# tkoolen/Parametron.jl

Hardware: AMD Instinct MI355X
Metric: QP re-evaluations/sec (Q,q,C,d rebuild) at n=4096 (higher is better)
Workload: dtype f64; 1 GPU; C2 dense least-squares QP: n=4096 vars, A 4096x4096, m=512 equality rows, fp64; canonical Q,q,const + C,d MOI triplets; n=4096, r=4096, m=512, objective_mode=canonical, instances_per_gpu=1, parallelism=single GPU, replay=tape

## Files before the change

### parametron.jl_amd/csrc/gram_mid.hip

```cpp
#include "affine_tile.h"
#include "gram_common.h"

#ifndef PMT_MID_WPS
#define PMT_MID_WPS 1
#endif
#ifndef PMT_MID_G
#define PMT_MID_G 256
#endif
#ifndef PMT_MID_MAXWG
#define PMT_MID_MAXWG 2304
#endif
#ifndef PMT_MID_D
#define PMT_MID_D 2
#endif
#ifndef PMT_MID_GROUP_US
#define PMT_MID_GROUP_US 1.15
#endif
#ifndef PMT_MID_TAIL_US
#define PMT_MID_TAIL_US 0.95
#endif
#ifndef PMT_MID_SB
#define PMT_MID_SB 8
#endif
#ifndef PMT_MID_FB
#define PMT_MID_FB 4
#endif
#ifndef PMT_MID_FORMAL
#if defined(__HIP_DEVICE_COMPILE__) && !defined(__gfx950__) && !defined(__gfx942__)
#define PMT_MID_FORMAL 1
#else
#define PMT_MID_FORMAL 0
#endif
#endif

#ifdef PMT_MID_TRACE
__device__ unsigned long long g_mid_trace[1024 * 8];
__device__ unsigned long long g_mid_walk[1024 * 8];
__device__ unsigned long long g_mid_riders[1024 * 2];
#define MID_TRACE_WORDS 8
__device__ __forceinline__ void mid_walk_note(unsigned long long *w, int k, unsigned long long t) {
    if (k == 0) { if (w[0]) w[4] += t - w[7]; else w[5] = t; w[0] += 1; }
    else if (k == 1) w[1] += t - w[7];
    else if (k == 3 || k == 5) { w[2] += t - w[7]; w[6] = t; }
    else if (k == 6) { w[3] += t - w[7]; w[6] = t; }
    else return;
    w[7] = t;
}
#define MID_STAMP(k) do { if (threadIdx.x == 0 && blockIdx.x < 1024) { const unsigned long long t_ = wall_clock64(); g_mid_trace[blockIdx.x * 8 + (k)] = t_; \
                          mid_walk_note(reinterpret_cast<unsigned long long *>(sh + MSH), (k), t_); } } while (0)
extern "C" int pmt_mid_trace_read(unsigned long long *host) {
    return hipMemcpyFromSymbol(host, HIP_SYMBOL(g_mid_trace), sizeof(unsigned long long) * 1024 * 8) == hipSuccess ? 0 : 1;
}
extern "C" int pmt_mid_walk_read(unsigned long long *host) {
    return hipMemcpyFromSymbol(host, HIP_SYMBOL(g_mid_walk), sizeof(unsigned long long) * 1024 * 8) == hipSuccess ? 0 : 1;
}
extern "C" int pmt_mid_riders_read(unsigned long long *host) {
    return hipMemcpyFromSymbol(host, HIP_SYMBOL(g_mid_riders), sizeof(unsigned long long) * 1024 * 2) == hipSuccess ? 0 : 1;
}
#else
#define MID_STAMP(k) do { } while (0)
#define MID_TRACE_WORDS 0
#endif

namespace pmt {

constexpr int MT = 64;
constexpr int MACC = 64;
constexpr int MPART = MACC * 64;
constexpr int MSTRIDE = MPART + MT + 8;
constexpr int MPITCH = MT + 1;
constexpr int MFG = 8;
constexpr int MCNT = 16;
constexpr int MQBUF = 4 * 2048;
constexpr int MFLAG = MQBUF + 4 * MT;
constexpr int MMAPS = MFLAG + 8;
constexpr int MSH = MMAPS + 2 * MT;

struct MidArgs {
    const double *A; int64_t lda, rows, cols;
    const double *b; int sign;
    const int64_t *xvar; const int64_t *varmap; int moi;
    QT *out_quad; double *out_csc; double alpha; LT *out_lin; double *out_const;
    int nb;
    int n_off, s_off, s_diag;
    int gpc_off, gpc_diag;
    int n_tail, s_tail, gpc_tail;
    double *ws;
    unsigned *counters;
    int xcd;
    int persist, total;
    unsigned *tickets;
    const AffineRider *riders;
    int nriders, rider_tiles;
};

struct MidPlan { int nb, n_off, s_off, s_diag, gpc_off, gpc_diag, n_tail, s_tail, gpc_tail, wgs; };

static double mid_fold_us(int count) { return 0.5 + 2.6 * (double)cdiv(count, PMT_MID_FB); }

static MidPlan mid_plan(int64_t rows, int64_t cols) {
    MidPlan p;
    p.nb = (int)cdiv(cols, MT);
    p.n_off = p.nb * (p.nb - 1) / 2;
    const int ngroups = (int)std::max<int64_t>(1, cdiv(rows, 8));
    const int maxs = std::max(1, ngroups / 4);
    auto sd = [&](int s) { return std::min(maxs, std::max(1, (5 * s + 7) / 8)); };
    int best = 1;
    double best_t = 1e300;
    for (int s = 1; s <= std::min(maxs, 64); ++s) {
        const int64_t wgs = (int64_t)p.n_off * s + (int64_t)p.nb * sd(s);
        if (s > 1 && wgs > PMT_MID_MAXWG) break;
        const double it_off = (double)cdiv(cdiv(ngroups, s), 4), it_diag = 0.69 * (double)cdiv(cdiv(ngroups, sd(s)), 4);
        const double fold = s <= 1 ? 0.0 : s <= MFG ? mid_fold_us(s) : mid_fold_us(MFG) + 1.5 + mid_fold_us((int)cdiv(s, MFG));
        const double t = (double)cdiv(wgs, PMT_MID_G) * (PMT_MID_GROUP_US * (p.n_off ? std::max(it_off, it_diag) : it_diag) + 5.0 + (s > 1 ? 1.0 : 0.0)) +
                         fold * (1.0 + (double)(p.n_off + p.nb) / PMT_MID_G);
        if (t < best_t) { best_t = t; best = s; }
    }
    int s = best;
#ifdef PMT_TUNING
    if (const char *e = getenv("PMT_MID_S")) { const int v = atoi(e); if (v > 0) s = std::min(v, maxs); }
#endif
    int sdiag = sd(s), ntail = 0, stail = 1;
    if (p.n_off + p.nb > PMT_MID_G) {
        auto wg_us = [&](int c, double w) { return PMT_MID_TAIL_US * w * (double)cdiv(cdiv(ngroups, c), 4) + 5.0 + (c > 1 ? 1.0 : 0.0); };
        const int rem = p.n_off % PMT_MID_G;
        int ct = 1;
        double tail_off = 0.0;
        if (rem) {
            tail_off = 1e300;
            for (int c = 1; c <= std::min(maxs, MFG); ++c) {
                const double t = (double)cdiv((int64_t)rem * c, PMT_MID_G) * wg_us(c, 1.0) + (c > 1 ? mid_fold_us(c) : 0.0);
                if (t < tail_off) { tail_off = t; ct = c; }
            }
        }
        const int last = rem ? (int)(((int64_t)rem * ct) % PMT_MID_G) : 0, free_cus = last ? PMT_MID_G - last : 0;
        const double t_last = rem ? wg_us(ct, 1.0) : wg_us(1, 1.0);
        int cd = 1;
        double tail_diag = 1e300;
        for (int c = 1; c <= std::min(maxs, MFG); ++c) {
            const double t_d = wg_us(c, 0.69);
            const int64_t inside = (int64_t)free_cus * (int64_t)(t_last / t_d);
            const int64_t left = std::max<int64_t>(0, (int64_t)p.nb * c - inside);
            const double t = (double)cdiv(left, PMT_MID_G) * t_d + (c > 1 ? mid_fold_us(c) : 0.0);
            if (t < tail_diag) { tail_diag = t; cd = c; }
        }
        const double t1 = (double)(p.n_off / PMT_MID_G) * wg_us(1, 1.0) + tail_off + tail_diag;
        if (s == 1 || t1 * (PMT_MID_GROUP_US / PMT_MID_TAIL_US) < best_t) { s = 1; sdiag = cd; ntail = ct > 1 ? rem : 0; stail = ct > 1 ? ct : 1; }
    }
#ifdef PMT_TUNING
    if (const char *e = getenv("PMT_MID_TAIL")) { if (atoi(e) == 0) { ntail = 0; stail = 1; } }
#endif
    p.gpc_off = (int)cdiv(ngroups, s);
    p.s_off = (int)cdiv(ngroups, p.gpc_off);
    p.gpc_diag = (int)cdiv(ngroups, sdiag);
    p.s_diag = (int)cdiv(ngroups, p.gpc_diag);
    p.n_tail = ntail;
    p.gpc_tail = (int)cdiv(ngroups, stail);
    p.s_tail = ntail ? (int)cdiv(ngroups, p.gpc_tail) : 1;
    if (p.s_tail <= 1) { p.n_tail = 0; p.s_tail = 1; p.gpc_tail = ngroups; }
    p.wgs = (p.n_off - p.n_tail) * p.s_off + p.n_tail * p.s_tail + p.nb * p.s_diag + 1;
    return p;
}

template <bool DIAG, bool FAST>
__device__ __forceinline__ void mid_load(const MidArgs &g, int64_t row0, int lane, int64_t cj0, int64_t ck0, const unsigned (&voff)[DIAG ? 4 : 8],
                                         f64x2 (&buf)[DIAG ? 4 : 8], f64x2 &cb) {
    constexpr int NG = DIAG ? 4 : 8;
    const int lm = lane & 15, lk = lane >> 4;
    if (FAST) {
        const char *base = reinterpret_cast<const char *>(g.A + row0);
#pragma unroll
        for (int t = 0; t < NG; ++t) buf[t] = *reinterpret_cast<const f64x2 *>(base + voff[t]);
        cb.x = 0.0; cb.y = 0.0;
        if (DIAG && g.b) cb = *reinterpret_cast<const f64x2 *>(g.b + row0 + 2 * lk);
        return;
    }
    const int64_t row = row0 + 2 * lk;
    const bool r0 = row < g.rows, r1 = row + 1 < g.rows;
#pragma unroll
    for (int t = 0; t < NG; ++t) {
        const int64_t col = (t < 4 ? cj0 : ck0) + 16 * (t & 3) + lm;
        const bool cv = col < g.cols;
        const bool v0 = cv && r0, v1 = cv && r1;
        const double *p0 = g.A + (v0 ? col * g.lda + row : 0), *p1 = g.A + (v1 ? col * g.lda + row + 1 : 0);
        const double x = *p0, y = *p1;
        buf[t].x = v0 ? x : 0.0;
        buf[t].y = v1 ? y : 0.0;
    }
    cb.x = 0.0; cb.y = 0.0;
    if (DIAG && g.b) {
        const double x = g.b[r0 ? row : 0], y = g.b[r1 ? row + 1 : 0];
        cb.x = r0 ? x : 0.0;
        cb.y = r1 ? y : 0.0;
    }
}

template <bool DIAG>
__device__ __forceinline__ void mid_compute(double *__restrict__ rot, const f64x2 (&buf)[DIAG ? 4 : 8], const f64x2 &cb, int sign, int lane,
                                            double (&acc)[MACC], double (&qacc)[4]) {
    constexpr int BO = DIAG ? 0 : 4;
    const int lm = lane & 15, lrow = lane & 48;
#pragma unroll
    for (int t = 0; t < 4; ++t) *reinterpret_cast<f64x2 *>(rot + (t * 64 + lane) * 2) = buf[BO + t];
    f64x2 bv[4][4];
#pragma unroll
    for (int c = 0; c < 4; ++c) {
        bv[c][0] = buf[BO + c];
#pragma unroll
        for (int r = 1; r < 4; ++r) {
            bv[c][r] = *reinterpret_cast<const f64x2 *>(rot + (c * 64 + lrow + ((lm + 4 * r) & 15)) * 2);
        }
    }
    __builtin_amdgcn_sched_barrier(0);
    constexpr int NC = 4;
#pragma unroll
    for (int c = 0; c < NC; ++c)
#pragma unroll
        for (int tm = 0; tm < (DIAG ? c + 1 : 4); ++tm) {
            const int a = (tm * 4 + c) * 4;
            acc[a] = __builtin_amdgcn_mfma_f64_4x4x4f64(buf[tm].x, bv[c][0].x, acc[a], 0, 0, 0);
        }
#pragma unroll
    for (int c = 0; c < NC; ++c)
#pragma unroll
        for (int tm = 0; tm < (DIAG ? c + 1 : 4); ++tm) {
            const int a = (tm * 4 + c) * 4;
            acc[a] = __builtin_amdgcn_mfma_f64_4x4x4f64(buf[tm].y, bv[c][0].y, acc[a], 0, 0, 0);
        }
    __builtin_amdgcn_sched_barrier(0);
#pragma unroll
    for (int c = 0; c < NC; ++c) {
#pragma unroll
        for (int r = 1; r < 4; ++r)
#pragma unroll
            for (int tm = 0; tm < (DIAG ? c + 1 : 4); ++tm) {
                const int a = (tm * 4 + c) * 4 + r;
                acc[a] = __builtin_amdgcn_mfma_f64_4x4x4f64(buf[tm].x, bv[c][r].x, acc[a], 0, 0, 0);
            }
#pragma unroll
        for (int r = 1; r < 4; ++r)
#pragma unroll
            for (int tm = 0; tm < (DIAG ? c + 1 : 4); ++tm) {
                const int a = (tm * 4 + c) * 4 + r;
                acc[a] = __builtin_amdgcn_mfma_f64_4x4x4f64(buf[tm].y, bv[c][r].y, acc[a], 0, 0, 0);
            }
    }
    if (DIAG) {
        const double c0 = signed_const(cb.x, sign), c1 = signed_const(cb.y, sign);
#pragma unroll
        for (int t = 0; t < 4; ++t) qacc[t] = __builtin_amdgcn_mfma_f64_4x4x4f64(buf[t].x, c0, qacc[t], 0, 0, 0);
#pragma unroll
        for (int t = 0; t < 4; ++t) qacc[t] = __builtin_amdgcn_mfma_f64_4x4x4f64(buf[t].y, c1, qacc[t], 0, 0, 0);
    }
}

#define MID_SB() __builtin_amdgcn_sched_barrier(0)
template <bool DIAG>
__device__ __forceinline__ void mid_step(const MidArgs &g, double *__restrict__ rot, int64_t next_row0, const char *base_a, const char *base_b,
                                         unsigned (&voff)[DIAG ? 4 : 8], f64x2 (&buf)[DIAG ? 4 : 8], f64x2 &cb, int sign, int lane,
                                         double (&acc)[MACC], double (&qacc)[4]) {
    constexpr int BO = DIAG ? 0 : 4;
    const int lm = lane & 15, lrow = lane & 48, lk = lane >> 4;
    auto reload = [&](int t) {
        asm volatile("" : "+v"(voff[t]));
        buf[t] = *reinterpret_cast<const f64x2 *>((t < 4 ? base_a : base_b) + voff[t]);
    };
    f64x2 bv[4][4];
#pragma unroll
    for (int c = 0; c < 4; ++c) bv[c][0] = buf[BO + c];
    auto lds_op = [&](int i) {
        if (i < 4) *reinterpret_cast<f64x2 *>(rot + (i * 64 + lane) * 2) = buf[BO + i];
        else {
            const int c = (i - 4) / 3, r = 1 + (i - 4) % 3;
            bv[c][r] = *reinterpret_cast<const f64x2 *>(rot + (c * 64 + lrow + ((lm + 4 * r) & 15)) * 2);
        }
    };
    MID_SB();
    int k = 0;
#pragma unroll
    for (int pass = 0; pass < 2; ++pass)
#pragma unroll
        for (int c = 0; c < 4; ++c)
#pragma unroll
            for (int tm = 0; tm < (DIAG ? c + 1 : 4); ++tm) {
                const int a = (tm * 4 + c) * 4;
                acc[a] = __builtin_amdgcn_mfma_f64_4x4x4f64(pass ? buf[tm].y : buf[tm].x, pass ? bv[c][0].y : bv[c][0].x, acc[a], 0, 0, 0);
                if (k < 16) { MID_SB(); lds_op(k); MID_SB(); }
                ++k;
            }
    if (DIAG) {
        const double c0 = signed_const(cb.x, sign), c1 = signed_const(cb.y, sign);
#pragma unroll
        for (int t = 0; t < 4; ++t) qacc[t] = __builtin_amdgcn_mfma_f64_4x4x4f64(buf[t].x, c0, qacc[t], 0, 0, 0);
#pragma unroll
        for (int t = 0; t < 4; ++t) qacc[t] = __builtin_amdgcn_mfma_f64_4x4x4f64(buf[t].y, c1, qacc[t], 0, 0, 0);
        MID_SB();
        cb = *reinterpret_cast<const f64x2 *>((g.b ? g.b : g.A) + next_row0 + 2 * lk);
    }
    MID_SB();
    int nb = 0;
#pragma unroll
    for (int tm = 0; tm < 4; ++tm) {
#pragma unroll
        for (int pass = 0; pass < 2; ++pass)
#pragma unroll
            for (int c = (DIAG ? tm : 0); c < 4; ++c)
#pragma unroll
                for (int r = 1; r < 4; ++r) {
                    const int a = (tm * 4 + c) * 4 + r;
                    acc[a] = __builtin_amdgcn_mfma_f64_4x4x4f64(pass ? buf[tm].y : buf[tm].x, pass ? bv[c][r].y : bv[c][r].x, acc[a], 0, 0, 0);
                    if (!DIAG && nb < 4) { MID_SB(); reload(4 + nb); MID_SB(); ++nb; }
                }
        MID_SB();
        reload(tm);
        MID_SB();
    }
}

__host__ __device__ constexpr bool mid_used(bool diag, int a) { return !diag || (a >> 4) <= ((a >> 2) & 3); }

__device__ __forceinline__ void mid_pos(int lane, int a, int &row, int &col) {
    const int i = lane >> 4, b = (lane >> 2) & 3, j = lane & 3;
    row = 16 * (a >> 4) + 4 * b + i;
    col = 16 * ((a >> 2) & 3) + 4 * ((b + (a & 3)) & 3) + j;
}

__device__ __forceinline__ void mid_maps(const MidArgs &g, double *sh, int tid, int jb, int kb) {
    u64 *cmap = reinterpret_cast<u64 *>(sh + MMAPS);
    if (tid >= 2 * MT || (!g.out_quad && jb != kb)) return;
    const int64_t i = (tid < MT ? (int64_t)kb * MT + tid : (int64_t)jb * MT + tid - MT);
    const int64_t v = i < g.cols ? g.xvar[i] : 1;
    cmap[tid] = (u64)(g.moi ? map_var(g.varmap, v) : v);
}

__device__ __forceinline__ void mid_epilogue(const MidArgs &g, double *sh, int tid, int jb, int kb) {
    const int wave = tid >> 6, lane = tid & 63;
    const int64_t n = g.cols, j0 = (int64_t)jb * MT, k0 = (int64_t)kb * MT;
    double *tile = sh;
    const double *qfin = sh + MT * MPITCH;
    const u64 *cmap = reinterpret_cast<const u64 *>(sh + MMAPS);
    const u64 *rmap = cmap + MT;
    if (g.out_csc) {
        const int64_t j = j0 + lane;
#pragma unroll 4
        for (int col = wave; col < MT; col += 4) {
            const int64_t k = k0 + col;
            double c = tile[lane * MPITCH + col];
            if (g.moi || j != k) c = 2 * c;
            if (k < n && j <= k) g.out_csc[k * (k + 1) / 2 + j] = g.alpha * c;
        }
    }
    if (g.out_quad) {
        u64 *out = reinterpret_cast<u64 *>(g.out_quad);
        u64 *desc = reinterpret_cast<u64 *>(sh + MT * MPITCH + MT);
        if (tid < MT) {
            const int64_t j = j0 + tid;
            const int64_t kstart = j > k0 ? j : k0;
            const int64_t kend = (k0 + MT < n) ? k0 + MT : n;
            const int64_t nterms = (j < n && kend > kstart) ? kend - kstart : 0;
            desc[2 * tid] = (u64)(j * n - (j * (j - 1)) / 2 + (kstart - j)) * 3;
            desc[2 * tid + 1] = (u64)nterms | (u64)(kstart - k0) << 16 | (u64)(kstart == j ? 1 : 0) << 24;
        }
        __syncthreads();
        const bool moi = g.moi != 0;
        const int uwave = __builtin_amdgcn_readfirstlane(wave);
#pragma unroll 4
        for (int i = 0; i < MT / 4; ++i) {
            const int row = 4 * i + uwave;
            const u64 w0 = desc[2 * row], info = desc[2 * row + 1];
            const int nterms = (int)(info & 0xffff), coff = (int)((info >> 16) & 0xff);
            const bool dg = ((info >> 24) & 1) != 0;
            double c = tile[row * MPITCH + coff + lane];
            const u64 m = cmap[(coff + lane) & (MT - 1)], rv = rmap[row];
            if (moi || !(dg && lane == 0)) c = 2 * c;
            if (lane < nterms) {
                u64 *d = out + w0 + 3 * lane;
                d[0] = (u64)__double_as_longlong(c);
                d[1] = rv;
                d[2] = m;
            }
        }
    }
    if (jb == kb && tid < MT) {
        const int64_t j = j0 + tid;
        if (j < n) {
            LT t;
            t.coeff = 2 * qfin[tid];
            t.var = (int64_t)rmap[tid];
            g.out_lin[j] = t;
        }
    }
}

__device__ __forceinline__ void mid_constant(const MidArgs &g, double *sh, int tid) {
    const int wave = tid >> 6, lane = tid & 63;
    double s0 = 0.0, s1 = 0.0;
    if (g.b && g.sign) {
        for (int64_t i = tid; i < g.rows; i += 512) { const double c = signed_const(g.b[i], g.sign); s0 = s0 + c * c; }
        for (int64_t i = tid + 256; i < g.rows; i += 512) { const double c = signed_const(g.b[i], g.sign); s1 = s1 + c * c; }
    }
#pragma unroll
    for (int off = 32; off > 0; off >>= 1) { s0 = s0 + __shfl_down(s0, off, 64); s1 = s1 + __shfl_down(s1, off, 64); }
    if (lane == 0) { sh[wave] = s0; sh[4 + wave] = s1; }
    __syncthreads();
    if (tid == 0) {
        double v = sh[0];
#pragma unroll
        for (int w = 1; w < 8; ++w) v = v + sh[w];
        *g.out_const = v;
    }
}

__device__ __forceinline__ void mid_put(double *p, double v) {
#if PMT_MID_FORMAL
    *p = v;
#else
    __hip_atomic_store(p, v, __ATOMIC_RELAXED, __HIP_MEMORY_SCOPE_AGENT);
#endif
}
__device__ __forceinline__ double mid_get(const double *p) {
#if PMT_MID_FORMAL
    return *p;
#else
    return __hip_atomic_load(p, __ATOMIC_RELAXED, __HIP_MEMORY_SCOPE_AGENT);
#endif
}

template <bool DIAG, int W>
__device__ __forceinline__ void mid_tail(const MidArgs &g, double *sh, int lane, double (&acc)[MACC], const double (&qacc)[4], int nchunk, double *w) {
    constexpr int KEEP1 = (W >> 1) * 32, GIVE1 = 32 - KEEP1, KEEP2 = KEEP1 + (W & 1) * 16, GIVE2 = KEEP1 + 16 - (W & 1) * 16;
    double *mine = sh + W * 2048;
    const double *half = sh + (W ^ 2) * 2048, *quarter = sh + (W ^ 1) * 2048;
    const bool qlane = (lane & 3) == 0;
    const int qcol = 4 * ((lane >> 2) & 3) + (lane >> 4);
#pragma unroll
    for (int a = 0; a < 32; a += 2)
        if (mid_used(DIAG, GIVE1 + a)) { f64x2 v; v.x = acc[GIVE1 + a]; v.y = acc[GIVE1 + a + 1]; *reinterpret_cast<f64x2 *>(mine + (a * 32 + lane) * 2) = v; }
    if (DIAG && qlane) {
#pragma unroll
        for (int t = 0; t < 4; ++t) sh[MQBUF + W * MT + 16 * t + qcol] = qacc[t];
    }
    __syncthreads();
#pragma unroll
    for (int a = 0; a < 32; a += 2)
        if (mid_used(DIAG, KEEP1 + a)) {
            const f64x2 v = *reinterpret_cast<const f64x2 *>(half + (a * 32 + lane) * 2);
            acc[KEEP1 + a] = acc[KEEP1 + a] + v.x; acc[KEEP1 + a + 1] = acc[KEEP1 + a + 1] + v.y;
        }
    double qsum = 0.0;
    if (DIAG && W == 0) qsum = (sh[MQBUF + lane] + sh[MQBUF + 2 * MT + lane]) + (sh[MQBUF + MT + lane] + sh[MQBUF + 3 * MT + lane]);
    __syncthreads();
#pragma unroll
    for (int a = 0; a < 16; a += 2)
        if (mid_used(DIAG, GIVE2 + a)) { f64x2 v; v.x = acc[GIVE2 + a]; v.y = acc[GIVE2 + a + 1]; *reinterpret_cast<f64x2 *>(mine + (a * 32 + lane) * 2) = v; }
    __syncthreads();
#pragma unroll
    for (int a = 0; a < 16; a += 2)
        if (mid_used(DIAG, KEEP2 + a)) {
            const f64x2 v = *reinterpret_cast<const f64x2 *>(quarter + (a * 32 + lane) * 2);
            acc[KEEP2 + a] = acc[KEEP2 + a] + v.x; acc[KEEP2 + a + 1] = acc[KEEP2 + a + 1] + v.y;
        }
    __syncthreads();
    if (nchunk == 1) {
#pragma unroll
        for (int a = KEEP2; a < KEEP2 + 16; ++a) {
            if (!mid_used(DIAG, a)) continue;
            int row, col;
            mid_pos(lane, a, row, col);
            sh[row * MPITCH + col] = acc[a];
        }
        if (DIAG && W == 0) sh[MT * MPITCH + lane] = qsum;
        return;
    }
#pragma unroll
    for (int a = KEEP2; a < KEEP2 + 16; ++a) if (mid_used(DIAG, a)) mid_put(&w[a * 64 + lane], acc[a]);
    if (DIAG && W == 0) mid_put(&w[MPART + lane], qsum);
#if PMT_MID_FORMAL
    __builtin_amdgcn_fence(__ATOMIC_RELEASE, "agent");
#else
    __builtin_amdgcn_s_waitcnt(0);
#endif
}

template <bool DIAG>
__device__ __forceinline__ void mid_fold(const double *p, int count, int64_t stride, int tid, double (&sum)[16], double &qs) {
#pragma unroll
    for (int u = 0; u < 16; ++u) sum[u] = 0.0;
    qs = 0.0;
    for (int c0 = 0; c0 < count; c0 += PMT_MID_FB) {
        double v[PMT_MID_FB][16], qv[PMT_MID_FB];
#pragma unroll
        for (int cc = 0; cc < PMT_MID_FB; ++cc) {
            const double *pc = p + (int64_t)min(c0 + cc, count - 1) * stride;
#pragma unroll
            for (int u = 0; u < 16; ++u) {
                const int a = (tid >> 6) + 4 * u;
                v[cc][u] = 0.0;
                if (mid_used(DIAG, a)) v[cc][u] = mid_get(pc + tid + 256 * u);
            }
            qv[cc] = 0.0;
            if (DIAG && tid < MT) qv[cc] = mid_get(pc + MPART + tid);
        }
#pragma unroll
        for (int cc = 0; cc < PMT_MID_FB; ++cc) {
            const bool live = c0 + cc < count;
#pragma unroll
            for (int u = 0; u < 16; ++u) { const double t = sum[u] + v[cc][u]; sum[u] = live ? t : sum[u]; }
            const double t = qs + qv[cc];
            qs = live ? t : qs;
        }
    }
}

struct MidWalk {
    bool early;
    unsigned *ticket; int id0;
    int *slot;
    int drawn;
    bool next_full; int njb, nkb, nrank;
    bool pre;
};

template <int N>
__device__ __forceinline__ void mid_forget(f64x2 (&buf)[PMT_MID_D][N]) {
#pragma unroll
    for (int d = 0; d < PMT_MID_D; ++d)
#pragma unroll
        for (int t = 0; t < N; ++t) asm volatile("" : "=v"(buf[d][t].x), "=v"(buf[d][t].y));
}

template <bool DIAG>
__device__ __forceinline__ auto &mid_buf(f64x2 (&own)[PMT_MID_D][4], f64x2 (&walk)[PMT_MID_D][8]) {
    if constexpr (DIAG) return own; else return walk;
}

template <bool DIAG, bool FAST>
__device__ __forceinline__ void mid_body(const MidArgs &g, double *sh, int tid, int jb, int kb, int chunk, int nchunk, int gpc, int first_wg, unsigned *counter,
                                         MidWalk &wk, f64x2 (&pbuf)[PMT_MID_D][8]) {
    constexpr int NG = DIAG ? 4 : 8;
    constexpr int D = PMT_MID_D;
    asm volatile("" : "+v"(tid));
    const int lane = tid & 63;
    const int wave = __builtin_amdgcn_readfirstlane(tid >> 6);
    const int lm = lane & 15, lk = lane >> 4;
    const int64_t cj0 = (int64_t)jb * MT, ck0 = (int64_t)kb * MT;
    const int ngroups = (int)((g.rows + 7) >> 3);
    const int g0 = chunk * gpc + wave, g1 = min((chunk + 1) * gpc, ngroups);
    const int my = g1 > g0 ? (g1 - g0 + 3) / 4 : 0;
    const bool ragged = FAST && (g.rows & 7) && my > 0 && g0 + 4 * (my - 1) == ngroups - 1;
    const int nfast = ragged ? my - 1 : my;

    MID_STAMP(0);
    mid_maps(g, sh, tid, jb, kb);
    double acc[MACC], qacc[4] = {0.0, 0.0, 0.0, 0.0};
#pragma unroll
    for (int a = 0; a < MACC; ++a) acc[a] = 0.0;
    unsigned voff[NG];
#pragma unroll
    for (int t = 0; t < NG; ++t) voff[t] = (unsigned)((min((t < 4 ? cj0 : ck0) + 16 * (t & 3) + lm, g.cols - 1) * g.lda + 2 * lk) * 8);
    double *rot = sh + wave * 512;
    f64x2 dbuf[D][4], cb[D];
    auto &buf = mid_buf<DIAG>(dbuf, pbuf);
    auto row_of = [&](int s) { return (int64_t)(g0 + 4 * min(s, max(nfast - 1, 0))) * 8; };
    const bool pre = !DIAG && wk.pre;
    bool pf = false;
    if (!DIAG && FAST) pf = wk.early && wk.next_full && nchunk == 1 && !ragged && nfast > 0 && nfast % D == 0 && (int64_t)(kb + 1) * MT <= g.cols;
    const int ahead_at = __builtin_amdgcn_readfirstlane(pf ? nfast - D : -1);
    const int64_t shift_a = pf ? ((int64_t)wk.njb * MT - cj0) * g.lda * 8 : 0, shift_b = pf ? ((int64_t)wk.nkb * MT - ck0) * g.lda * 8 : 0;
    if (nfast > 0) {
        if (!pre) {
#pragma unroll
            for (int d = 0; d < D; ++d) {
                __builtin_amdgcn_sched_barrier(0);
                mid_load<DIAG, FAST>(g, row_of(d), lane, cj0, ck0, voff, buf[d], cb[d]);
            }
            __builtin_amdgcn_sched_barrier(0);
        }
        if (FAST) {
            int s0 = 0;
            for (; s0 + D <= nfast; s0 += D) {
                const bool ahead = s0 == ahead_at;
#pragma unroll
                for (int d = 0; d < D; ++d) {
                    const int64_t row = ahead ? row_of(d) : row_of(s0 + d + D);
                    const char *base = reinterpret_cast<const char *>(g.A + row);
                    mid_step<DIAG>(g, rot, row, base + (ahead ? shift_a : 0), base + (ahead ? shift_b : 0), voff, buf[d], cb[d], g.sign, lane, acc, qacc);
                }
            }
#pragma unroll
            for (int d = 0; d < D - 1; ++d)
                if (s0 + d < nfast) mid_compute<DIAG>(rot, buf[d], cb[d], g.sign, lane, acc, qacc);
        } else {
            for (int s0 = 0; s0 < nfast; s0 += D) {
#pragma unroll
                for (int d = 0; d < D; ++d) {
                    if (s0 + d < nfast) mid_compute<DIAG>(rot, buf[d], cb[d], g.sign, lane, acc, qacc);
                    mid_load<DIAG, FAST>(g, row_of(s0 + d + D), lane, cj0, ck0, voff, buf[d], cb[d]);
                }
            }
        }
    }
    if (ragged) {
        mid_load<DIAG, false>(g, (int64_t)(ngroups - 1) * 8, lane, cj0, ck0, voff, buf[0], cb[0]);
        mid_compute<DIAG>(rot, buf[0], cb[0], g.sign, lane, acc, qacc);
    }

    MID_STAMP(1);
    wk.pre = pf;
    unsigned drawn = 0;
    if (!DIAG && wk.early && tid == 0) drawn = __hip_atomic_fetch_add(wk.ticket, 1u, __ATOMIC_RELAXED, __HIP_MEMORY_SCOPE_AGENT);
    unsigned *flag = reinterpret_cast<unsigned *>(sh + MFLAG);
    double *w = g.ws + (int64_t)(first_wg + chunk) * MSTRIDE;
    __syncthreads();
    if (wave == 0) mid_tail<DIAG, 0>(g, sh, lane, acc, qacc, nchunk, w);
    else if (wave == 1) mid_tail<DIAG, 1>(g, sh, lane, acc, qacc, nchunk, w);
    else if (wave == 2) mid_tail<DIAG, 2>(g, sh, lane, acc, qacc, nchunk, w);
    else mid_tail<DIAG, 3>(g, sh, lane, acc, qacc, nchunk, w);
    MID_STAMP(2);
    if (nchunk > 1) {
        const bool two = nchunk > MFG;
        const int gfirst = two ? (chunk / MFG) * MFG : 0;
        const int n1 = two ? min(MFG, nchunk - gfirst) : nchunk;
        unsigned *c1 = two ? counter + 1 + chunk / MFG : counter;
        __syncthreads();
        if (tid == 0) *flag = __hip_atomic_fetch_add(c1, 1u, __ATOMIC_RELAXED, __HIP_MEMORY_SCOPE_AGENT);
        __syncthreads();
        MID_STAMP(3);
        if (*flag != (unsigned)(n1 - 1)) { mid_forget(buf); return; }
#if PMT_MID_FORMAL
        __builtin_amdgcn_fence(__ATOMIC_ACQUIRE, "agent");
#endif
        if (tid == 0) __hip_atomic_store(c1, 0u, __ATOMIC_RELAXED, __HIP_MEMORY_SCOPE_AGENT);
        double sum[16], qs;
        double *p = g.ws + (int64_t)(first_wg + gfirst) * MSTRIDE;
        mid_fold<DIAG>(p, n1, MSTRIDE, tid, sum, qs);
        if (two) {
#pragma unroll
            for (int u = 0; u < 16; ++u) if (mid_used(DIAG, (tid >> 6) + 4 * u)) mid_put(p + tid + 256 * u, sum[u]);
            if (DIAG && tid < MT) mid_put(p + MPART + tid, qs);
#if PMT_MID_FORMAL
            __builtin_amdgcn_fence(__ATOMIC_RELEASE, "agent");
#else
            __builtin_amdgcn_s_waitcnt(0);
#endif
            __syncthreads();
            if (tid == 0) *flag = __hip_atomic_fetch_add(counter, 1u, __ATOMIC_RELAXED, __HIP_MEMORY_SCOPE_AGENT);
            __syncthreads();
            const int ng = (nchunk + MFG - 1) / MFG;
            if (*flag != (unsigned)(ng - 1)) { mid_forget(buf); return; }
#if PMT_MID_FORMAL
            __builtin_amdgcn_fence(__ATOMIC_ACQUIRE, "agent");
#endif
            if (tid == 0) __hip_atomic_store(counter, 0u, __ATOMIC_RELAXED, __HIP_MEMORY_SCOPE_AGENT);
            mid_fold<DIAG>(g.ws + (int64_t)first_wg * MSTRIDE, ng, (int64_t)MFG * MSTRIDE, tid, sum, qs);
        }
        __syncthreads();
        MID_STAMP(4);
#pragma unroll
        for (int u = 0; u < 16; ++u) {
            const int a = (tid >> 6) + 4 * u;
            if (!mid_used(DIAG, a)) continue;
            int row, col;
            mid_pos(lane, a, row, col);
            sh[row * MPITCH + col] = sum[u];
        }
        if (DIAG && tid < MT) sh[MT * MPITCH + tid] = qs;
        mid_forget(buf);
    }
    if (!DIAG && wk.early && tid == 0) *wk.slot = wk.id0 + 8 * (int)drawn;
    __syncthreads();
    if (!DIAG && wk.early) wk.drawn = *wk.slot;
    MID_STAMP(5);
    mid_epilogue(g, sh, tid, jb, kb);
#ifdef PMT_MID_TRACE
    __builtin_amdgcn_s_waitcnt(0);
    MID_STAMP(6);
#endif
}

__device__ __forceinline__ int mid_xcd_rank(int id, int base, int n) {
    const int x = id & 7, end = base + n;
    int start = 0;
    for (int y = 0; y < x; ++y) {
        const int fy = base + ((y - base) & 7);
        start += fy < end ? ((end - 1 - fy) >> 3) + 1 : 0;
    }
    return start + ((id - (base + ((x - base) & 7))) >> 3);
}

__device__ __forceinline__ void mid_tile_of(int t, int nb, int &jb, int &kb) {
    constexpr int SB = PMT_MID_SB;
    const int nsb = (nb + SB - 1) / SB;
    for (int K = 0; K < nsb; ++K) {
        const int wK = min(SB, nb - SB * K);
        for (int J = 0; J <= K; ++J) {
            const int cnt = J < K ? SB * wK : wK * (wK - 1) / 2;
            if (t >= cnt) { t -= cnt; continue; }
            if (J < K) { jb = SB * J + t / wK; kb = SB * K + t % wK; return; }
            int kk = 1;
            while (t >= kk) { t -= kk; ++kk; }
            jb = SB * K + t; kb = SB * K + kk;
            return;
        }
    }
    jb = 0; kb = 1;
}

struct MidItem { int kind, jb, kb, chunk, nch, gpc, first, rank; };
__device__ __forceinline__ MidItem mid_decode(const MidArgs &g, int id) {
    MidItem it = {2, 0, 0, 0, 1, 0, 0, 0};
    const int nbody = g.n_off - g.n_tail, wbody = nbody * g.s_off, noff = wbody + g.n_tail * g.s_tail;
    if (id < noff) {
        const bool tail = id >= wbody;
        const int base = tail ? wbody : 0, ntile = tail ? g.n_tail : nbody, nch = tail ? g.s_tail : g.s_off;
        const int k = g.xcd ? mid_xcd_rank(id, base, ntile * nch) : ((id - base) % nch) * ntile + (id - base) / nch;
        const int chunk = k / ntile;
        const int rank = (tail ? nbody : 0) + (k - chunk * ntile);
        int t = rank, jb, kb;
        if (g.xcd) mid_tile_of(t, g.nb, jb, kb);
        else {
            kb = 1;
            while (t >= kb) { t -= kb; ++kb; }
            jb = t;
        }
        it.kind = 0; it.jb = jb; it.kb = kb; it.chunk = chunk; it.nch = nch; it.gpc = tail ? g.gpc_tail : g.gpc_off;
        it.first = tail ? wbody + (rank - nbody) * g.s_tail : rank * g.s_off;
        it.rank = rank;
        return it;
    }
    if (id < noff + g.nb * g.s_diag) {
        const int k = g.xcd ? mid_xcd_rank(id, noff, g.nb * g.s_diag) : ((id - noff) % g.s_diag) * g.nb + (id - noff) / g.s_diag;
        const int chunk = k / g.nb, jb = k - chunk * g.nb;
        it.kind = 1; it.jb = jb; it.kb = jb; it.chunk = chunk; it.nch = g.s_diag; it.gpc = g.gpc_diag; it.first = noff + jb * g.s_diag; it.rank = g.n_off + jb;
    }
    return it;
}

template <bool FAST>
__device__ __forceinline__ void mid_item(const MidArgs &g, double *sh, int tid, const MidItem &it, MidWalk &wk, f64x2 (&pbuf)[PMT_MID_D][8]) {
    if (it.kind == 0) {
        mid_body<false, FAST>(g, sh, tid, it.jb, it.kb, it.chunk, it.nch, it.gpc, it.first, g.counters + it.rank * MCNT, wk, pbuf);
        return;
    }
    wk.pre = false;
    if (it.kind == 1) mid_body<true, FAST>(g, sh, tid, it.jb, it.kb, it.chunk, it.nch, it.gpc, it.first, g.counters + it.rank * MCNT, wk, pbuf);
    else mid_constant(g, sh, tid);
    mid_forget(pbuf);
}

__device__ __forceinline__ void mid_rider_tile(const AffineRider &r, int local, double *sh) {
    int t;
    asm volatile("v_mov_b32 %0, %1" : "=v"(t) : "v"((int)threadIdx.x));
    const int by = local / r.tiles_x, bx = local - by * r.tiles_x;
    double *tile = sh;
    u64 *vmx = reinterpret_cast<u64 *>(sh + TILE * PITCH);
#define MID_RIDE(NTV, TRV, NTLV)                                                                                                         \
    affine_tile_body<1, NTV, TRV, NTLV>(r.A, r.lda, r.rows, r.cols, r.xvar, r.b, r.sign, r.varmap, r.row_offset, r.out, r.out_consts,   \
                                        r.vec_in, r.vec_out, bx, by, t, tile, vmx)
    if (r.ntl) { if (r.tr == 32) MID_RIDE(true, 32, true); else MID_RIDE(true, 64, true); }
#ifdef PMT_TUNING
    else if (!r.nt) { if (r.tr == 32) MID_RIDE(false, 32, false); else MID_RIDE(false, 64, false); }
#endif
    else { if (r.tr == 32) MID_RIDE(true, 32, false); else MID_RIDE(true, 64, false); }
#undef MID_RIDE
}
static_assert(TILE * PITCH + TILE <= MQBUF, "a rider's tile and its variable-map row live in the front of the kernel's LDS");

template <bool FAST>
__global__ __launch_bounds__(256, PMT_MID_WPS) void gram_mid_kernel(MidArgs g) {
    __shared__ double sh[MSH + MID_TRACE_WORDS];
    __shared__ int next_id, ahead_id;
    const int tid = threadIdx.x;
    const int x = blockIdx.x & 7, per = gridDim.x >> 3;
#ifdef PMT_MID_TRACE
    if (tid == 0) for (int i = 0; i < MID_TRACE_WORDS; ++i) reinterpret_cast<unsigned long long *>(sh + MSH)[i] = 0;
#endif
    f64x2 pbuf[PMT_MID_D][8];
    MidWalk wk = {};
    wk.ticket = g.tickets + x; wk.id0 = x + 8 * per; wk.slot = &ahead_id;
    const int wbody = (g.n_off - g.n_tail) * g.s_off;
    const bool look = FAST && g.persist && g.s_off == 1;
    int id = blockIdx.x, hand = -1;
    if (look) {
        if (tid == 0) next_id = wk.id0 + 8 * (int)__hip_atomic_fetch_add(wk.ticket, 1u, __ATOMIC_RELAXED, __HIP_MEMORY_SCOPE_AGENT);
        __syncthreads();
        hand = next_id;
    }
    MidItem cur = mid_decode(g, id);
    for (;;) {
        wk.early = hand >= 0 && hand < wbody;
        wk.next_full = false;
        if (wk.early) {
            const MidItem nx = mid_decode(g, hand);
            wk.next_full = (int64_t)(nx.kb + 1) * MT <= g.cols;
            wk.njb = nx.jb; wk.nkb = nx.kb; wk.nrank = nx.rank;
        }
        mid_item<FAST>(g, sh, tid, cur, wk, pbuf);
        if (!g.persist) return;
        __syncthreads();
        if (wk.early) {
            id = hand; hand = wk.drawn;
            cur.jb = wk.njb; cur.kb = wk.nkb; cur.first = cur.rank = wk.nrank;
            continue;
        }
        if (hand >= 0) { id = hand; hand = -1; }
        else {
            if (tid == 0) next_id = wk.id0 + 8 * (int)__hip_atomic_fetch_add(wk.ticket, 1u, __ATOMIC_RELAXED, __HIP_MEMORY_SCOPE_AGENT);
            __syncthreads();
            id = next_id;
        }
        if (id >= g.total) break;
        cur = mid_decode(g, id);
    }
    if (g.rider_tiles > 0) {
        int mine = 0;
        for (;;) {
            __syncthreads();
            if (tid == 0) next_id = (int)__hip_atomic_fetch_add(g.tickets + 9, 1u, __ATOMIC_RELAXED, __HIP_MEMORY_SCOPE_AGENT);
            __syncthreads();
            const int rt = __builtin_amdgcn_readfirstlane(next_id);
            if (rt >= g.rider_tiles) break;
            int k = 0;
            while (k + 1 < g.nriders && rt >= g.riders[k + 1].first_tile) ++k;
            mid_rider_tile(g.riders[k], rt - g.riders[k].first_tile, sh);
            ++mine;
        }
#ifdef PMT_MID_TRACE
        __builtin_amdgcn_s_waitcnt(0);
        if (tid == 0 && blockIdx.x < 1024) { g_mid_riders[blockIdx.x * 2] = (unsigned long long)mine; g_mid_riders[blockIdx.x * 2 + 1] = wall_clock64(); }
#endif
        (void)mine;
    }
#ifdef PMT_MID_TRACE
    if (tid == 0 && blockIdx.x < 1024) {
        for (int i = 0; i < 7; ++i) g_mid_walk[blockIdx.x * 8 + i] = reinterpret_cast<unsigned long long *>(sh + MSH)[i];
        g_mid_walk[blockIdx.x * 8 + 7] = wall_clock64();
    }
#endif
    if (tid == 0) {
        const unsigned gone = __hip_atomic_fetch_add(g.tickets + 8, 1u, __ATOMIC_RELAXED, __HIP_MEMORY_SCOPE_AGENT);
        if (gone == gridDim.x - 1) {
#pragma unroll
            for (int i = 0; i < 10; ++i) __hip_atomic_store(g.tickets + i, 0u, __ATOMIC_RELAXED, __HIP_MEMORY_SCOPE_AGENT);
        }
    }
}

__global__ __launch_bounds__(256) void gram_mid_constant_kernel(MidArgs g) {
    __shared__ double sh[8];
    mid_constant(g, sh, threadIdx.x);
}
int launch_gram_mid_constant(const double *b, int sign, int64_t rows, double *out_const, hipStream_t s) {
    MidArgs g = {};
    g.rows = rows; g.b = (b && sign) ? b : nullptr; g.sign = g.b ? sign : 0; g.out_const = out_const;
    PMT_LAUNCH_NAMED("gram_mid_constant_kernel", gram_mid_constant_kernel, dim3(1), dim3(256), 0, s, g);
    return check_launch("gram_mid_constant_kernel");
}

size_t gram_mid_workspace_bytes(int64_t rows, int64_t cols) {
    if (cols <= 0) return 0;
    const MidPlan p = mid_plan(rows, cols);
    return sizeof(double) * (size_t)p.wgs * MSTRIDE;
}
bool gram_mid_persistent(int64_t rows, int64_t cols) { return cols > 0 && rows > 0 && mid_plan(rows, cols).wgs >= 2 * PMT_MID_G; }
int gram_mid_counters(int64_t cols) { const int nb = (int)cdiv(cols, MT); return MCNT * (nb * (nb + 1) / 2) + 16; }

int launch_gram_mid(const double *A, int64_t lda, int64_t rows, int64_t cols, const int64_t *xvar, const double *b, int sign, int moi,
                    const int64_t *varmap, pmt_quadratic_term *out_quad, double *out_csc, double alpha, pmt_linear_term *out_lin,
                    double *out_const, void *workspace, unsigned *counters, const void *riders, int nriders, int rider_tiles, hipStream_t s) {
    if (!workspace || !counters) return fail(PMT_INVALID_ARGUMENT, "quad_gram: workspace required");
    const MidPlan p = mid_plan(rows, cols);
    MidArgs g;
    g.A = A; g.lda = lda; g.rows = rows; g.cols = cols; g.b = (b && sign) ? b : nullptr; g.sign = g.b ? sign : 0;
    g.xvar = xvar; g.varmap = varmap; g.moi = moi; g.out_quad = reinterpret_cast<QT *>(out_quad); g.out_csc = out_csc; g.alpha = alpha;
    g.out_lin = reinterpret_cast<LT *>(out_lin); g.out_const = out_const;
    g.nb = p.nb; g.n_off = p.n_off; g.s_off = p.s_off; g.s_diag = p.s_diag; g.gpc_off = p.gpc_off; g.gpc_diag = p.gpc_diag;
    g.n_tail = p.n_tail; g.s_tail = p.s_tail; g.gpc_tail = p.gpc_tail;
    g.ws = reinterpret_cast<double *>(workspace); g.counters = counters;
    g.xcd = rows * cols * 8 > ((int64_t)4 << 20);
    const bool fast = (reinterpret_cast<uintptr_t>(A) & 15) == 0 && (lda & 1) == 0 && (reinterpret_cast<uintptr_t>(g.b) & 15) == 0 &&
                      (uint64_t)lda * (uint64_t)cols * 8 < (1ull << 32);
    g.total = p.wgs;
    g.persist = p.wgs >= 2 * PMT_MID_G;
    g.tickets = counters + gram_mid_counters(cols) - 16;
    const bool ride = g.persist && riders && nriders > 0 && rider_tiles > 0;
    g.riders = ride ? static_cast<const AffineRider *>(riders) : nullptr; g.nriders = ride ? nriders : 0; g.rider_tiles = ride ? rider_tiles : 0;
    const unsigned grid = g.persist ? (unsigned)PMT_MID_G : (unsigned)p.wgs;
    if (fast) PMT_LAUNCH_NAMED("gram_mid_kernel", (gram_mid_kernel<true>), dim3(grid), dim3(256), 0, s, g);
    else PMT_LAUNCH_NAMED("gram_mid_kernel", (gram_mid_kernel<false>), dim3(grid), dim3(256), 0, s, g);
    return check_launch("gram_mid_kernel");
}

}
```

Measured before the change: 893.2 re-evaluations/s.

## Replace two-stage LDS butterfly reduction with single all-to-all exchange in mid tail

The cross-wave accumulator reduction in mid_tail now writes each wave's non-owned 16-slot quarters to dedicated LDS pieces in one pass, then each wave reads its three incoming pieces and sums them. This replaces the two butterfly rounds and removes three of the four barriers. The final tile, qfin and descriptor regions are moved to separate LDS offsets so they no longer alias the exchange buffers, which also lets the post-fold syncthreads go. In exchange the kernel uses more LDS (12 pieces instead of 4 halves) and holds more registers for the staged reads, which may lower occupancy. It also adds small address-space and inline-asm hints on the ticket atomic and the slot store.

```diff
diff --git a/parametron.jl_amd/csrc/gram_mid.hip b/parametron.jl_amd/csrc/gram_mid.hip
--- a/parametron.jl_amd/csrc/gram_mid.hip
+++ b/parametron.jl_amd/csrc/gram_mid.hip
@@ -71,10 +71,15 @@
 constexpr int MPITCH = MT + 1;
 constexpr int MFG = 8;
 constexpr int MCNT = 16;
-constexpr int MQBUF = 4 * 2048;
+constexpr int MXPIECE = 16 * 64;
+constexpr int MQBUF = 12 * MXPIECE;
 constexpr int MFLAG = MQBUF + 4 * MT;
 constexpr int MMAPS = MFLAG + 8;
-constexpr int MSH = MMAPS + 2 * MT;
+constexpr int MTILE = MMAPS + 2 * MT;
+constexpr int MQFIN = MTILE + MT * MPITCH;
+constexpr int MDESC = MQFIN + MT;
+constexpr int MSH = MDESC + 2 * MT;
+static_assert((MSH + 16) * sizeof(double) <= 160 * 1024, "gfx950: 160 KiB of LDS per CU");
 
 struct MidArgs {
     const double *A; int64_t lda, rows, cols;
@@ -336,8 +341,7 @@
 __device__ __forceinline__ void mid_epilogue(const MidArgs &g, double *sh, int tid, int jb, int kb) {
     const int wave = tid >> 6, lane = tid & 63;
     const int64_t n = g.cols, j0 = (int64_t)jb * MT, k0 = (int64_t)kb * MT;
-    double *tile = sh;
-    const double *qfin = sh + MT * MPITCH;
+    const double *tile = sh + MTILE, *qfin = sh + MQFIN;
     const u64 *cmap = reinterpret_cast<const u64 *>(sh + MMAPS);
     const u64 *rmap = cmap + MT;
     if (g.out_csc) {
@@ -352,7 +356,7 @@
     }
     if (g.out_quad) {
         u64 *out = reinterpret_cast<u64 *>(g.out_quad);
-        u64 *desc = reinterpret_cast<u64 *>(sh + MT * MPITCH + MT);
+        u64 *desc = reinterpret_cast<u64 *>(sh + MDESC);
         if (tid < MT) {
             const int64_t j = j0 + tid;
             const int64_t kstart = j > k0 ? j : k0;
@@ -428,52 +432,56 @@
 
 template <bool DIAG, int W>
 __device__ __forceinline__ void mid_tail(const MidArgs &g, double *sh, int lane, double (&acc)[MACC], const double (&qacc)[4], int nchunk, double *w) {
-    constexpr int KEEP1 = (W >> 1) * 32, GIVE1 = 32 - KEEP1, KEEP2 = KEEP1 + (W & 1) * 16, GIVE2 = KEEP1 + 16 - (W & 1) * 16;
-    double *mine = sh + W * 2048;
-    const double *half = sh + (W ^ 2) * 2048, *quarter = sh + (W ^ 1) * 2048;
+    constexpr int OWN = 16 * W;
+    auto piece = [&](int owner, int giver) { return sh + MXPIECE * (3 * owner + (giver ^ owner) - 1); };
     const bool qlane = (lane & 3) == 0;
     const int qcol = 4 * ((lane >> 2) & 3) + (lane >> 4);
 #pragma unroll
-    for (int a = 0; a < 32; a += 2)
-        if (mid_used(DIAG, GIVE1 + a)) { f64x2 v; v.x = acc[GIVE1 + a]; v.y = acc[GIVE1 + a + 1]; *reinterpret_cast<f64x2 *>(mine + (a * 32 + lane) * 2) = v; }
+    for (int o = 0; o < 4; ++o) {
+        if (o == W) continue;
+        double *to = piece(o, W);
+#pragma unroll
+        for (int a = 0; a < 16; a += 2)
+            if (mid_used(DIAG, 16 * o + a)) { f64x2 v; v.x = acc[16 * o + a]; v.y = acc[16 * o + a + 1]; *reinterpret_cast<f64x2 *>(to + (a * 32 + lane) * 2) = v; }
+    }
     if (DIAG && qlane) {
 #pragma unroll
         for (int t = 0; t < 4; ++t) sh[MQBUF + W * MT + 16 * t + qcol] = qacc[t];
     }
     __syncthreads();
-#pragma unroll
-    for (int a = 0; a < 32; a += 2)
-        if (mid_used(DIAG, KEEP1 + a)) {
-            const f64x2 v = *reinterpret_cast<const f64x2 *>(half + (a * 32 + lane) * 2);
-            acc[KEEP1 + a] = acc[KEEP1 + a] + v.x; acc[KEEP1 + a + 1] = acc[KEEP1 + a + 1] + v.y;
-        }
+    const double *p2 = piece(W, W ^ 2), *p1 = piece(W, W ^ 1), *p3 = piece(W, W ^ 3);
+    f64x2 v1[8], v2[8], v3[8];
+#pragma unroll
+    for (int i = 0; i < 8; ++i) {
+        if (!mid_used(DIAG, OWN + 2 * i)) continue;
+        v2[i] = *reinterpret_cast<const f64x2 *>(p2 + (i * 64 + lane) * 2);
+        v1[i] = *reinterpret_cast<const f64x2 *>(p1 + (i * 64 + lane) * 2);
+        v3[i] = *reinterpret_cast<const f64x2 *>(p3 + (i * 64 + lane) * 2);
+    }
+    __builtin_amdgcn_sched_barrier(0);
+#pragma unroll
+    for (int i = 0; i < 8; ++i) {
+        const int a = OWN + 2 * i;
+        if (!mid_used(DIAG, a)) continue;
+        acc[a] = (acc[a] + v2[i].x) + (v1[i].x + v3[i].x);
+        acc[a + 1] = (acc[a + 1] + v2[i].y) + (v1[i].y + v3[i].y);
+    }
+    __builtin_amdgcn_sched_barrier(0);
     double qsum = 0.0;
     if (DIAG && W == 0) qsum = (sh[MQBUF + lane] + sh[MQBUF + 2 * MT + lane]) + (sh[MQBUF + MT + lane] + sh[MQBUF + 3 * MT + lane]);
-    __syncthreads();
-#pragma unroll
-    for (int a = 0; a < 16; a += 2)
-        if (mid_used(DIAG, GIVE2 + a)) { f64x2 v; v.x = acc[GIVE2 + a]; v.y = acc[GIVE2 + a + 1]; *reinterpret_cast<f64x2 *>(mine + (a * 32 + lane) * 2) = v; }
-    __syncthreads();
-#pragma unroll
-    for (int a = 0; a < 16; a += 2)
-        if (mid_used(DIAG, KEEP2 + a)) {
-            const f64x2 v = *reinterpret_cast<const f64x2 *>(quarter + (a * 32 + lane) * 2);
-            acc[KEEP2 + a] = acc[KEEP2 + a] + v.x; acc[KEEP2 + a + 1] = acc[KEEP2 + a + 1] + v.y;
-        }
-    __syncthreads();
     if (nchunk == 1) {
 #pragma unroll
-        for (int a = KEEP2; a < KEEP2 + 16; ++a) {
+        for (int a = OWN; a < OWN + 16; ++a) {
             if (!mid_used(DIAG, a)) continue;
             int row, col;
             mid_pos(lane, a, row, col);
-            sh[row * MPITCH + col] = acc[a];
-        }
-        if (DIAG && W == 0) sh[MT * MPITCH + lane] = qsum;
+            sh[MTILE + row * MPITCH + col] = acc[a];
+        }
+        if (DIAG && W == 0) sh[MQFIN + lane] = qsum;
         return;
     }
 #pragma unroll
-    for (int a = KEEP2; a < KEEP2 + 16; ++a) if (mid_used(DIAG, a)) mid_put(&w[a * 64 + lane], acc[a]);
+    for (int a = OWN; a < OWN + 16; ++a) if (mid_used(DIAG, a)) mid_put(&w[a * 64 + lane], acc[a]);
     if (DIAG && W == 0) mid_put(&w[MPART + lane], qsum);
 #if PMT_MID_FORMAL
     __builtin_amdgcn_fence(__ATOMIC_RELEASE, "agent");
@@ -608,7 +616,11 @@
     MID_STAMP(1);
     wk.pre = pf;
     unsigned drawn = 0;
-    if (!DIAG && wk.early && tid == 0) drawn = __hip_atomic_fetch_add(wk.ticket, 1u, __ATOMIC_RELAXED, __HIP_MEMORY_SCOPE_AGENT);
+    if (!DIAG && wk.early && tid == 0) {
+        auto *ticket = (__attribute__((address_space(1))) unsigned *)wk.ticket;
+        asm volatile("" : "+v"(ticket));
+        drawn = __hip_atomic_fetch_add(ticket, 1u, __ATOMIC_RELAXED, __HIP_MEMORY_SCOPE_AGENT);
+    }
     unsigned *flag = reinterpret_cast<unsigned *>(sh + MFLAG);
     double *w = g.ws + (int64_t)(first_wg + chunk) * MSTRIDE;
     __syncthreads();
@@ -654,7 +666,6 @@
             if (tid == 0) __hip_atomic_store(counter, 0u, __ATOMIC_RELAXED, __HIP_MEMORY_SCOPE_AGENT);
             mid_fold<DIAG>(g.ws + (int64_t)first_wg * MSTRIDE, ng, (int64_t)MFG * MSTRIDE, tid, sum, qs);
         }
-        __syncthreads();
         MID_STAMP(4);
 #pragma unroll
         for (int u = 0; u < 16; ++u) {
@@ -662,12 +673,16 @@
             if (!mid_used(DIAG, a)) continue;
             int row, col;
             mid_pos(lane, a, row, col);
-            sh[row * MPITCH + col] = sum[u];
-        }
-        if (DIAG && tid < MT) sh[MT * MPITCH + tid] = qs;
+            sh[MTILE + row * MPITCH + col] = sum[u];
+        }
+        if (DIAG && tid < MT) sh[MQFIN + tid] = qs;
         mid_forget(buf);
     }
-    if (!DIAG && wk.early && tid == 0) *wk.slot = wk.id0 + 8 * (int)drawn;
+    if (!DIAG && wk.early && tid == 0) {
+        int stride = 8;
+        asm volatile("" : "+s"(stride));
+        *wk.slot = wk.id0 + stride * (int)drawn;
+    }
     __syncthreads();
     if (!DIAG && wk.early) wk.drawn = *wk.slot;
     MID_STAMP(5);
```

Result: no change. 895.7 re-evaluations/s, median of 6 (+0.3%).
